# Idokorro/MiniGrid-RL

Hardware: AMD Instinct MI355X
Metric: env-steps/sec at 65k parallel envs, 1/2/4/8 MI355X; % HBM roofline (higher is better)
Workload: dtype u8

## Files before the change

### minigrid-rl_amd/csrc/mgx_device.h

```cpp
#pragma once
#ifndef MGX_HOST_SIM
#include <hip/hip_runtime.h>
#else
#include "host_sim.h"
#endif
#include <stdint.h>

#include "mgx_diag.h"

namespace mgx {

constexpr uint8_t CODE_EMPTY = 0x01;
constexpr uint8_t CODE_WALL = 2 | (5 << 4);
constexpr uint8_t CODE_GOAL = 8 | (1 << 4);
constexpr uint8_t CODE_LAVA = 9;
constexpr int T_EMPTY = 1, T_WALL = 2, T_DOOR = 4, T_KEY = 5, T_BALL = 6, T_BOX = 7,
              T_GOAL = 8, T_LAVA = 9, T_OPEN = 11;
constexpr int A_LEFT = 0, A_RIGHT = 1, A_FORWARD = 2, A_PICKUP = 3, A_DROP = 4,
              A_TOGGLE = 5, A_DONE = 6;
constexpr uint8_t NONE8 = 0xFF;

__device__ __forceinline__ int cn2idx(int cn) { return (0x403512 >> (cn * 4)) & 0xF; }

__device__ __forceinline__ uint8_t mk_code(int t, int cidx, int aux) {
// ... 276 lines not shown
#else
#define GCOUNT(G, k) do { } while (0)
#endif
#endif


template <int NW>
__device__ __forceinline__ void put(Gen<NW> &G, int x, int y, uint8_t code) {
    const int b = y * G.S + x;
    G.g[b] = code;
    if (code == CODE_EMPTY) G.occ.unset(b); else G.occ.set(b);
}

#ifndef MGX_HOST_SIM
typedef __attribute__((address_space(3))) uint64_t lds_u64;
#else
typedef uint64_t lds_u64;
#endif
constexpr int MT_PAD = MT_WG_MAX + 4;
template <int WG>
__device__ __noinline__ void mt_refill_cold(const uint64_t *__restrict__ table, uint64_t slot, lds_u64 *win) {
    const uint4 *src = reinterpret_cast<const uint4 *>(table + slot);
    static_assert(WG % 8 == 0 && WG <= MT_WG_MAX, "window loads go in fours of 16 B");
#pragma unroll
    for (int h = 0; h < WG / 8; h++) {
        const uint4 v0 = src[4 * h], v1 = src[4 * h + 1], v2 = src[4 * h + 2], v3 = src[4 * h + 3];
        lds_u64 *d = win + 8 * h;
        d[0] = (uint64_t)v0.x | ((uint64_t)v0.y << 32); d[1] = (uint64_t)v0.z | ((uint64_t)v0.w << 32);
        d[2] = (uint64_t)v1.x | ((uint64_t)v1.y << 32); d[3] = (uint64_t)v1.z | ((uint64_t)v1.w << 32);
        d[4] = (uint64_t)v2.x | ((uint64_t)v2.y << 32); d[5] = (uint64_t)v2.z | ((uint64_t)v2.w << 32);
        d[6] = (uint64_t)v3.x | ((uint64_t)v3.y << 32); d[7] = (uint64_t)v3.z | ((uint64_t)v3.w << 32);
    }
}
template <int NW>
__device__ __forceinline__ uint64_t win_group(Gen<NW> &G, uint64_t g) {
    constexpr int MT_WG = mt_wg<NW>();
    uint64_t off = g - G.gbase;
    if (off >= MT_WG) {
        GCOUNT(G, 23);
        if (g < G.tlo || g + MT_WG > G.thi) G.err |= 1u;
        mt_refill_cold<MT_WG>(G.table, g & G.rmask, (lds_u64 *)G.win);
        G.gbase = g;
        off = 0;
    }
    return G.win[off];
}
__device__ __forceinline__ uint64_t div10(uint64_t v) { return __umul64hi(v, 0xCCCCCCCCCCCCCCCDull) >> 3; }
template <int NW>
__device__ __forceinline__ void mt_sync(Gen<NW> &G) {
    const uint64_t g = div10(G.cur);
    G.go = (int)(G.cur - g * MT_FIELDS);
    G.gi = g;
    G.ga = win_group(G, g);
    G.gb = win_group(G, g + 1);
    G.gc = win_group(G, g + 2);
}
struct RbConst {
    uint64_t c1;
    uint32_t sh;
};
__device__ __forceinline__ RbConst rb_const(uint32_t n) {
    const uint32_t sh = 5u - (uint32_t)(32 - __clz(n));
    return RbConst{(uint64_t)(32u + (n << sh) - 1u) * MT_REP, sh};
}
template <int NW>
__device__ __forceinline__ int randbelow_c(Gen<NW> &G, const RbConst K);
template <int NW>
__device__ __forceinline__ int randbelow(Gen<NW> &G, uint32_t n) {
    GCOUNT(G, 24);
    if (n >= 32u) { G.err |= 8u; return 0; }
    return randbelow_c(G, rb_const(n));
}
template <int NW>
__device__ __forceinline__ int randbelow_c(Gen<NW> &G, const RbConst K) {
    const uint64_t c1 = K.c1;
    const uint32_t sh = K.sh;
    for (;;) {
        GCOUNT(G, 21);
        const int o6 = (int)__umul24((uint32_t)G.go, 6u);
        const uint64_t f = ((G.ga >> o6) | (G.gb << (60 - o6))) & MT_LOW60;
        const uint64_t acc = (c1 - f) & (32ull * MT_REP);
        const uint32_t left = G.llw - (uint32_t)(G.cur - G.astart);
        const int j = acc ? (int)(((uint32_t)__ffsll((long long)acc) - 1u - 5u) * 171u >> 10) : MT_FIELDS;
        int m = j < MT_FIELDS ? j + 1 : MT_FIELDS;
        if ((uint32_t)m > left) {
            G.cur = G.astart + G.llw;
            G.abort = true;
            return 0;
        }
        const int r = (int)(((f >> (6 * (j < MT_FIELDS ? j : 0))) & 31u) >> sh);
        G.cur += (uint64_t)m;
        G.go += m;
        if (G.go >= MT_FIELDS) {
            G.go -= MT_FIELDS;
            G.ga = G.gb;
            G.gb = G.gc;
            G.gi++;
            G.gc = win_group(G, G.gi + 2);
        }
        if (j < MT_FIELDS) return r;
    }
}
template <class GT>
__device__ __forceinline__ void mt_advance(GT &G, int m) {
    G.cur += (uint64_t)m;
    G.go += m;
    if (G.go >= MT_FIELDS) {
        G.go -= MT_FIELDS;
        G.ga = G.gb;
        G.gb = G.gc;
        G.gi++;
        G.gc = win_group(G, G.gi + 2);
    }
}
template <class GT>
__device__ __forceinline__ uint64_t randbelow_seq(GT &G, uint64_t prog, int cnt) {
    constexpr uint64_t GM = 32ull * MT_REP;
    uint64_t res = 0;
    int i = 0;
#pragma unroll 1
    while (i < cnt) {
        GCOUNT(G, 21);
        const int o6 = (int)__umul24((uint32_t)G.go, 6u);
        const uint64_t f = ((G.ga >> o6) | (G.gb << (60 - o6))) & MT_LOW60;
        uint64_t avail = GM;
        int used = MT_FIELDS;
#pragma unroll 1
        while (i < cnt) {
            const RbConst K = rb_const((uint32_t)(prog >> (5 * i)) & 31u);
            const uint64_t acc = (K.c1 - f) & avail;
            if (!acc) { used = MT_FIELDS; break; }
            const int b = __ffsll((long long)acc) - 1;
            res |= (uint64_t)((((uint32_t)(f >> (b - 5))) & 31u) >> K.sh) << (5 * i);
            avail &= ~((2ull << b) - 1ull);
            used = (int)((uint32_t)(b + 1) * 171u >> 10);
            i++;
        }
        const uint32_t left = G.llw - (uint32_t)(G.cur - G.astart);
        if ((uint32_t)used > left) {
            G.cur = G.astart + G.llw;
            G.abort = true;
            return res;
        }
        mt_advance(G, used);
    }
    return res;
}
__device__ __forceinline__ uint32_t guard10(uint64_t acc) {
    constexpr uint32_t K = (1u << 20) | (1u << 15) | (1u << 10) | (1u << 5) | 1u;
    const uint32_t lo = (uint32_t)acc >> 5, hi = (uint32_t)(acc >> 32) >> 3;
    return (((lo * K) >> 20) & 31u) | ((((hi * K) >> 20) & 31u) << 5);
}
template <int NW, typename Bad, typename Sat>
__device__ __forceinline__ void draw_cell(Gen<NW> &G, const RbConst KX, const RbConst KY, int x0, int y0, int &x, int &y,
                                          Bad bad, Sat sat ,
                                          bool has_c, const RbConst KC, int &choice) {
    constexpr uint64_t GM = 32ull * MT_REP;
    int rej = 0;
    bool need_c = has_c, have_x = false;
    uint32_t xv = 0;
#pragma unroll 1
    for (;;) {
        GCOUNT(G, 27);
        GCOUNT(G, 21);
        const int o6 = (int)__umul24((uint32_t)G.go, 6u);
        const uint64_t f = ((G.ga >> o6) | (G.gb << (60 - o6))) & MT_LOW60;
        uint32_t avail = 0x3FFu;
        if (need_c) {
            const uint32_t mc = guard10((KC.c1 - f) & GM);
            const uint32_t j = (uint32_t)__builtin_ctz(mc | 0x400u);
            choice = mc ? (int)((((uint32_t)(f >> (6u * j))) & 31u) >> KC.sh) : choice;
            avail &= ~1u << j;
            need_c = mc == 0u;
        }
        const uint32_t mx = guard10((KX.c1 - f) & GM), my = guard10((KY.c1 - f) & GM);
        bool ok;
        uint32_t jy;
#pragma unroll 1
        for (;;) {
            GCOUNT(G, 25);
            const uint32_t cx = mx & avail;
            const uint32_t jx = (uint32_t)__builtin_ctz(cx | 0x400u);
            const uint32_t xn = (((uint32_t)(f >> (6u * jx))) & 31u) >> KX.sh;
            const uint32_t av = have_x ? avail : avail & (~1u << jx);
            xv = have_x ? xv : xn;
            const uint32_t cy = my & av;
            jy = (uint32_t)__builtin_ctz(cy | 0x400u);
            x = x0 + (int)xv;
            y = y0 + (int)((((uint32_t)(f >> (6u * jy))) & 31u) >> KY.sh);
            avail = av & (~1u << jy);
            have_x = cy == 0u && (have_x || cx != 0u);
            ok = cy != 0u && !bad(x, y);
            if (ok || cy == 0u) break;
            if (++rej == SAT_PROBE && !sat()) { live_lock(G); return; }
        }
        const int used = ok ? (int)jy + 1 : MT_FIELDS;
        const uint32_t left = G.llw - (uint32_t)(G.cur - G.astart);
        if ((uint32_t)used > left) {
            G.cur = G.astart + G.llw;
            G.abort = true;
            return;
        }
        G.cur += (uint64_t)used;
        G.go += used;
        const bool rot = G.go >= MT_FIELDS;
        G.go -= rot ? MT_FIELDS : 0;
        G.ga = rot ? G.gb : G.ga;
        G.gb = rot ? G.gc : G.gb;
        G.gi += rot ? 1ull : 0ull;
        G.gc = win_group(G, G.gi + 2);
        if (ok) return;
    }
}

template <int NW>
__device__ __forceinline__ int randint(Gen<NW> &G, int a, int b) { return a + randbelow(G, (uint32_t)(b - a + 1)); }
template <int NW>
__device__ __forceinline__ bool choice_bool(Gen<NW> &G) { return randbelow(G, 2) == 0; }

template <int NW>
__device__ __forceinline__ bool next2door(const Gen<NW> &G, int x, int y) {
    if constexpr (NW == 4) {
        return is_door(G.g[y * G.S + x - 1]) || is_door(G.g[y * G.S + x + 1]) ||
               is_door(G.g[(y - 1) * G.S + x]) || is_door(G.g[(y + 1) * G.S + x]);
    } else {
        return G.dn.test(y * G.S + x);
    }
}
template <int NW>
__device__ __forceinline__ bool occupied(const Gen<NW> &G, int b) {
    if constexpr (NW == 4) return G.g[b] != CODE_EMPTY;
    else return G.occ.test(b);
}

constexpr uint32_t OBJ_KEYFLAG = 1u << 24;
template <int NW>
__device__ __forceinline__ void add_obj(Gen<NW> &G, int t, int cname, int x, int y, uint32_t flags = 0) {
    const bool full = G.nobjs >= MAX_OBJS;
    G.err |= full ? 8u : 0u;
    G.tmask |= full ? 0u : 1u << t;
    const bool first_goal = !full && t == T_GOAL && G.goalx < 0;
    G.goalx = first_goal ? x : G.goalx;
    G.goaly = first_goal ? y : G.goaly;
    if (!full)
        G.objs[G.nobjs++] = (uint32_t)t | ((uint32_t)(cname & 15) << 4) | ((uint32_t)x << 8) | ((uint32_t)y << 16) | flags;
}

template <int NW>
__device__ __forceinline__ void draw_free_cell(Gen<NW> &G, int &px, int &py) {
    for (uint32_t it = 0;; ++it) {
        GCOUNT(G, 22);
        if (it > PCG_LOOP_LIMIT) { G.err |= 4u; px = 1; py = 1; return; }
        int x, y;
        pcg_cell(G.pcg, G.S, x, y);
        if (occupied(G, y * G.S + x)) continue;
        if (x == G.ax && y == G.ay) continue;
        px = x; py = y;
        return;
    }
}
template <int NW>
__device__ __forceinline__ void place_agent(Gen<NW> &G) {
    G.ax = -1; G.ay = -1;
    int x, y;
    draw_free_cell(G, x, y);
    G.ax = x; G.ay = y;
    G.adir = pcg_integers(G.pcg, 0, 4);
}

__device__ __forceinline__ int nth_set_bit(uint32_t m, int r) {
    int pos = 0, c;
    c = __popc(m & 0xFFFFu); if (r >= c) { r -= c; m >>= 16; pos += 16; }
    c = __popc(m & 0xFFu);   if (r >= c) { r -= c; m >>= 8;  pos += 8; }
    c = __popc(m & 0xFu);    if (r >= c) { r -= c; m >>= 4;  pos += 4; }
    c = __popc(m & 0x3u);    if (r >= c) { r -= c; m >>= 2;  pos += 2; }
    c = (int)(m & 1u);       if (r >= c) { pos += 1; }
    return pos;
}
template <int NW>
__device__ __forceinline__ int mask_choice(Gen<NW> &G, uint32_t m) {
    return nth_set_bit(m, randbelow(G, (uint32_t)__popc(m)));
}

template <int NW>
__device__ __forceinline__ void live_lock(Gen<NW> &G) {
    G.cur = G.astart + G.llw;
    G.abort = true;
}

template <int NW>
__device__ __forceinline__ void place_key(Gen<NW> &G, int x0, int x1, int y0, int y1, int gx, int gy, bool chk_agent,
                                          int ox, int oy, int cname, bool kib, int *kx, int *ky) {
    int x, y, rej = 0;
    for (;;) {
        x = randint(G, x0, x1);
        y = randint(G, y0, y1);
        if (G.abort) return;
        const bool bad = (x == gx && y == gy) || (chk_agent && x == G.ax && y == G.ay) || (x == ox && y == oy) ||
                         next2door(G, x, y);
        if (!bad) break;
        if (++rej == SAT_PROBE) {
            bool sat = false;
            for (int xx = x0; xx <= x1 && !sat; xx++)
                for (int yy = y0; yy <= y1 && !sat; yy++)
                    sat = !((xx == gx && yy == gy) || (chk_agent && xx == G.ax && yy == G.ay) ||
                            (xx == ox && yy == oy) || next2door(G, xx, yy));
            if (!sat) { live_lock(G); return; }
        }
    }
    const int cidx = cn2idx(cname);
    if (kib) { put(G, x, y, mk_code(T_BOX, cidx, 1)); add_obj(G, T_BOX, cname, x, y, OBJ_KEYFLAG); }
    else { put(G, x, y, mk_code(T_KEY, cidx, 0)); add_obj(G, T_KEY, cname, x, y, OBJ_KEYFLAG); }
    if (kx) { *kx = x; *ky = y; }
}

template <int NW>
__device__ __forceinline__ void place_objects(Gen<NW> &G, uint32_t &oc, const int *types, int n, int x0, int x1,
                                              int y0, int y1) {
    for (int k = 0; k < n; k++) {
        if (oc == 0) { G.err |= 8u; return; }
        const int b = mask_choice(G, oc);
        if (G.abort) return;
        oc &= ~(1u << b);
        const int t = types[b / 6], cname = b % 6;
        int x, y, rej = 0;
        for (;;) {
            x = randint(G, x0, x1);
            y = randint(G, y0, y1);
            if (G.abort) return;
            const bool bad = occupied(G, y * G.S + x) || (x == G.ax && y == G.ay) || next2door(G, x, y);
            if (!bad) break;
            if (++rej == SAT_PROBE) {
                bool sat = false;
                for (int xx = x0; xx <= x1 && !sat; xx++)
                    for (int yy = y0; yy <= y1 && !sat; yy++)
                        sat = !(occupied(G, yy * G.S + xx) || (xx == G.ax && yy == G.ay) || next2door(G, xx, yy));
                if (!sat) { live_lock(G); return; }
            }
        }
        put(G, x, y, mk_code(t, cn2idx(cname), 0));
        add_obj(G, t, cname, x, y);
    }
}

__device__ __forceinline__ int door_code(int cname, bool locked, bool open) {
    return open ? mk_code(T_OPEN, cn2idx(cname), 0) : mk_code(T_DOOR, cn2idx(cname), locked ? 1 : 0);
}

template <int NW>
__device__ __forceinline__ void put_door(Gen<NW> &G, int x, int y, uint8_t code) {
    put(G, x, y, code);
    const int S = G.S, b = y * S + x;
    if (x > 0) G.dn.set(b - 1);
    if (x < S - 1) G.dn.set(b + 1);
    if (y > 0) G.dn.set(b - S);
    if (y < S - 1) G.dn.set(b + S);
}

template <int NW>
__device__ __forceinline__ uint32_t bits_row(const Bits<NW> &B, int y, int S) {
    const int b = y * S;
    uint64_t v = b < 64 ? (B.w0 >> b) : 0ull;
    if (NW > 1) {
        if (b >= 64) v = B.w1 >> (b - 64);
        else if (b + S > 64) v |= B.w1 << (64 - b);
    }
    return (uint32_t)v & ((1u << S) - 1u);
}
template <int NW>
__device__ __forceinline__ bool rect_has_free(const Gen<NW> &G, int x0, int x1, int y0, int y1, bool use_occ,
                                              int ax, int ay, int bx, int by, int cx, int cy) {
    if constexpr (NW == 4) {
        return true;
    } else {
        const uint32_t rowmask = ((1u << (x1 - x0 + 1)) - 1u) << x0;
        bool sat = false;
        for (int y = y0; y <= y1; y++) {
            uint32_t bad = bits_row(G.dn, y, G.S);
            if (use_occ) bad |= bits_row(G.occ, y, G.S);
            if (ay == y && ax >= 0) bad |= 1u << ax;
            if (by == y && bx >= 0) bad |= 1u << bx;
            if (cy == y && cx >= 0) bad |= 1u << cx;
            sat |= (rowmask & ~bad) != 0;
        }
        return sat;
    }
}


__device__ __forceinline__ void door_geom(int nr, int d, int mid, int S, bool &horiz, int &lo, int &hi) {
    if (nr == 2) { horiz = false; lo = 1; hi = S - 2; return; }
    if (nr == 3) {
        horiz = d == 0;
        lo = d == 2 ? mid + 1 : 1;
        hi = d == 2 ? S - 2 : mid - 1;
        return;
    }
    horiz = d < 2;
    const bool upper_half = (d == 0 || d == 2);
    lo = upper_half ? 1 : mid + 1;
    hi = upper_half ? mid - 1 : S - 2;
}

__device__ __forceinline__ int room_of(int nr, int x, int y, int mid) {
    const bool left = x < mid, up = y < mid;
    if (nr == 2) return left ? 0 : 1;
    if (nr == 3) return left ? (up ? 0 : 1) : 2;
    return left ? (up ? 0 : 1) : (up ? 2 : 3);
}

__device__ __forceinline__ void room_rect(int nr, int r, int mid, int S, int &x0, int &x1, int &y0, int &y1) {
    const bool left = (nr == 2) ? r == 0 : r <= 1;
    const bool full_h = nr == 2 || (nr == 3 && r == 2);
    const bool up = (r == 0) || (nr == 4 && r == 2);
    x0 = left ? 1 : mid + 1; x1 = left ? mid - 1 : S - 2;
    y0 = full_h ? 1 : (up ? 1 : mid + 1); y1 = full_h ? S - 2 : (up ? mid - 1 : S - 2);
}

__device__ __forceinline__ void key_spec(int nr, int r, int ar, int &kA, int &kB, bool &chk) {
    kA = -1; kB = -1; chk = (r == ar);
    if (nr == 2) { if (r == ar) kA = 0; return; }
    if (nr == 3) {
        if (r != ar) return;
        if (r == 0) { kA = 1; kB = 0; }
        else if (r == 1) { kA = 2; kB = 0; }
        else { kA = 2; kB = 1; }
        return;
    }
    const int HL = 0, HR = 1, VU = 2, VL = 3;
    if (r == 0) {
        if (ar == 0) { kA = VU; kB = HL; } else if (ar == 1) kA = VU; else if (ar == 2) kA = HL;
    } else if (r == 1) {
        if (ar == 1) { kA = VL; kB = HL; } else if (ar == 3) kA = HL; else if (ar == 0) kA = VL;
    } else if (r == 2) {
        if (ar == 2) { kA = VU; kB = HR; } else if (ar == 3) kA = VU; else if (ar == 0) kA = HR;
    } else {
        if (ar == 3) { kA = VL; kB = HR; } else if (ar == 1) kA = HR; else if (ar == 2) kA = VL;
    }
}

__device__ const int MULTI_TYPES[3] = {T_KEY, T_BALL, T_BOX};

struct Prefix {
    int nr, rc;
    uint32_t dinfo;
    uint32_t dpos;
    uint32_t dopen;
};
template <class GT>
__device__ __forceinline__ void prefix_draws(GT &G, int S, bool draw_cmd, bool ado, Prefix &P) {
    const uint64_t r = randbelow_seq(G, draw_cmd ? (4ull | (3ull << 5)) : 3ull, draw_cmd ? 2 : 1);
    P.rc = draw_cmd ? (int)(r & 31) : 0;
    P.nr = 2 + (int)((draw_cmd ? r >> 5 : r) & 31);
    P.dinfo = P.dpos = P.dopen = 0;
    if (G.abort || (MGX_GEN_SKIP & 8)) return;
    const int nr = P.nr, mid = S / 2, ndoors = nr == 2 ? 1 : nr;
    uint64_t prog = 0;
    int cnt = 0;
#pragma unroll 1
    for (int d = 0; d < ndoors; d++) {
        prog |= (uint64_t)(6 - d) << (5 * cnt++);
        if (!ado) prog |= 2ull << (5 * cnt++);
        prog |= 2ull << (5 * cnt++);
    }
    const uint64_t dr = randbelow_seq(G, prog, cnt);
    if (G.abort) return;
    uint32_t dc = 0x3Fu;
#pragma unroll 1
    for (int d = 0, k = 0; d < ndoors; d++) {
        const int col = nth_set_bit(dc, (int)(dr >> (5 * k++)) & 31);
        dc &= ~(1u << col);
        const bool lk = ado ? false : ((dr >> (5 * k++)) & 31) == 0;
        const bool kib = ((dr >> (5 * k++)) & 31) == 0;
        P.dinfo |= (uint32_t)(col | (lk << 3) | (kib << 4)) << (8 * d);
    }
    prog = 0;
    cnt = 0;
#pragma unroll 1
    for (int d = 0; d < ndoors; d++) {
        bool horiz; int lo, hi;
        door_geom(nr, d, mid, S, horiz, lo, hi);
        prog |= (uint64_t)(hi - lo + 1) << (5 * cnt++);
        if (ado) prog |= 2ull << (5 * cnt++);
    }
    const uint64_t pr = randbelow_seq(G, prog, (MGX_GEN_SKIP & 2) ? 0 : cnt);
    if (G.abort) return;
#pragma unroll 1
    for (int d = 0, k = 0; d < ((MGX_GEN_SKIP & 2) ? 0 : ndoors); d++) {
        P.dpos |= (uint32_t)((pr >> (5 * k++)) & 15) << (4 * d);
        if (ado) P.dopen |= (uint32_t)(((pr >> (5 * k++)) & 31) == 0) << d;
    }
}
constexpr int PFX_LOOK = 320;
__host__ __device__ __forceinline__ uint64_t pfx_pack(const Prefix &P, uint32_t adv, uint32_t tag) {
    uint64_t r = (uint64_t)(adv & 0xFF) | ((uint64_t)(tag & 0xFF) << 8) | ((uint64_t)(P.nr - 2) << 16) |
                 ((uint64_t)(P.rc & 3) << 18);
    for (int d = 0; d < 4; d++)
        r |= (uint64_t)(((P.dinfo >> (8 * d)) & 31) | (((P.dpos >> (4 * d)) & 15) << 5) | (((P.dopen >> d) & 1) << 9))
             << (20 + 10 * d);
    return r;
}
__host__ __device__ __forceinline__ void pfx_unpack(uint64_t r, Prefix &P) {
    P.nr = 2 + (int)((r >> 16) & 3);
    P.rc = (int)((r >> 18) & 3);
    P.dinfo = P.dpos = P.dopen = 0;
    for (int d = 0; d < 4; d++) {
        const uint32_t f = (uint32_t)(r >> (20 + 10 * d)) & 0x3FFu;
        P.dinfo |= (f & 31u) << (8 * d);
        P.dpos |= ((f >> 5) & 15u) << (4 * d);
        P.dopen |= ((f >> 9) & 1u) << d;
    }
}
constexpr int MT_SB_WORDS = 3120;
constexpr int MT_SB_GROUPS = MT_SB_WORDS / MT_FIELDS;
constexpr int MT_SLIDE_MAX_SB = 64;
__host__ __device__ __forceinline__ int mt_slide_superblocks(unsigned long long hi, unsigned long long need_lo,
                                                             unsigned long long want_hi,
                                                             unsigned long long ring_groups) {
    int nsb = 0;
    while (nsb < MT_SLIDE_MAX_SB && hi + (unsigned long long)nsb * MT_SB_GROUPS < want_hi &&
           hi + (unsigned long long)(nsb + 1) * MT_SB_GROUPS <= need_lo + ring_groups)
        nsb++;
    return nsb;
}
struct PfxWindow {
    unsigned long long zero_lo, rec_lo, rec_hi;
    unsigned long long next_done;
    unsigned long long strides;
};
__host__ __device__ __forceinline__ PfxWindow pfx_window(unsigned long long rec_done, unsigned long long hi,
                                                         unsigned long long ring_words, unsigned long long threads,
                                                         unsigned long long look) {
    const unsigned long long top = hi * (unsigned long long)MT_FIELDS;
    const unsigned long long held = top > ring_words ? top - ring_words : 0ull;
    PfxWindow w;
    w.rec_hi = top > look ? top - look : 0ull;
    w.rec_lo = rec_done > held ? rec_done : held;
    if (w.rec_hi < w.rec_lo) w.rec_hi = w.rec_lo;
    w.zero_lo = w.rec_lo;
    if (rec_done < held) {
        const unsigned long long kept = w.rec_hi > ring_words ? w.rec_hi - ring_words : 0ull;
        w.zero_lo = rec_done > kept ? rec_done : kept;
    }
    w.next_done = w.rec_hi;
    w.strides = (w.rec_hi - w.rec_lo + threads - 1) / threads;
    return w;
}

template <int NW>
__device__ __forceinline__ void gen_rooms(Gen<NW> &G, const Prefix &P) {
    const int S = G.S, mid = S / 2, nr = P.nr;
    if (MGX_GEN_SKIP & 8) { G.ax = 1; G.ay = 1; put(G, S - 2, S - 2, CODE_GOAL); add_obj(G, T_GOAL, 15, S - 2, S - 2); return; }
    for (int i = 1; i < S - 1; i++) put(G, mid, i, CODE_WALL);
    if (nr == 3) for (int i = 1; i < mid; i++) put(G, i, mid, CODE_WALL);
    if (nr == 4) for (int i = 1; i < S - 1; i++) put(G, i, mid, CODE_WALL);
    const int ndoors = nr == 2 ? 1 : nr;
    const bool ado = G.all_doors_open;
    const uint32_t dinfo = P.dinfo;
    uint32_t oc = 0x3FFFFu;
#pragma unroll 1
    for (int d = 0; d < ndoors; d++) {
        const uint32_t di = dinfo >> (8 * d);
        const int col = di & 7;
        if ((di >> 3) & 1) { oc &= ~(1u << col); if ((di >> 4) & 1) oc &= ~(1u << (12 + col)); }
    }
    GSTAMP(G, 11);
#pragma unroll 1
    for (int d = 0; d < ((MGX_GEN_SKIP & 2) ? 0 : ndoors); d++) {
        bool horiz; int lo, hi;
        door_geom(nr, d, mid, S, horiz, lo, hi);
        const int v = lo + (int)((P.dpos >> (4 * d)) & 15);
        const int x = horiz ? v : mid, y = horiz ? mid : v;
        const uint32_t di = dinfo >> (8 * d);
        const bool open = ado && ((P.dopen >> d) & 1);
        put_door(G, x, y, (uint8_t)door_code(di & 7, (di >> 3) & 1, open));
        add_obj(G, T_DOOR, di & 7, x, y);
    }
    GSTAMP(G, 12);
    if (G.abort) return;
    int gx = 1, gy = 1;
    if (MGX_GEN_SKIP & 4) {
        gx = 1; gy = 1; put(G, gx, gy, CODE_GOAL); add_obj(G, T_GOAL, 15, gx, gy); G.ax = S - 2; G.ay = S - 2;
    } else {
        bool agent = false;
        int gcell = -1;
        if constexpr (NW <= 2) {
#pragma unroll 1
            for (uint32_t it = 0;; ++it) {
                GCOUNT(G, 22);
                if (it > 2 * PCG_LOOP_LIMIT) { G.err |= 4u; G.ax = 1; G.ay = 1; break; }
                int x, y;
                pcg_cell(G.pcg, S, x, y);
                const int b = y * S + x;
                Bits<NW> rejm = G.occ;
                rejm.w0 |= agent ? 0ull : G.dn.w0;
                if (NW > 1) rejm.w1 |= agent ? 0ull : G.dn.w1;
                if (rejm.test(b)) continue;
                if (agent) { G.ax = x; G.ay = y; break; }
                gx = x; gy = y; gcell = b;
                G.occ.set(b);
                agent = true;
            }
        } else {
#pragma unroll 1
            for (uint32_t it = 0;; ++it) {
                GCOUNT(G, 22);
                if (it > 2 * PCG_LOOP_LIMIT) { G.err |= 4u; G.ax = 1; G.ay = 1; break; }
                int x, y;
                pcg_cell(G.pcg, S, x, y);
                const int b = y * S + x;
                if (occupied(G, b) || b == gcell) continue;
                if (agent) { G.ax = x; G.ay = y; break; }
                if (next2door(G, x, y)) continue;
                gx = x; gy = y; gcell = b;
                agent = true;
            }
        }
        if (gcell >= 0) {
            put(G, gx, gy, CODE_GOAL);
            add_obj(G, T_GOAL, 15, gx, gy);
        }
        G.adir = pcg_integers(G.pcg, 0, 4);
    }
    GSTAMP(G, 13);
    const int gr = room_of(nr, gx, gy, mid), ar = room_of(nr, G.ax, G.ay, mid);
    const int n_left = G.num_objects / 2, n_right = G.num_objects - n_left;
    int c0, c1, c2, c3;
    if (nr == 2) { c0 = n_left; c1 = n_right; c2 = c3 = 0; }
    else if (nr == 3) { c0 = n_left / 2; c1 = n_left - c0; c2 = n_right; c3 = 0; }
    else { c0 = n_left / 2; c1 = n_left - c0; c2 = n_right / 2; c3 = n_right - c2; }
    uint32_t keymask = 0;
    uint32_t npack = 0;
    uint32_t kspec = 0;
#pragma unroll
    for (int r = 0; r < 4; r++) {
        int kA, kB;
        bool chk;
        key_spec(nr, r, ar, kA, kB, chk);
        kspec |= (uint32_t)(kA & 3) << (4 * r) | (uint32_t)(kB & 3) << (4 * r + 2) | (uint32_t)chk << (16 + r);
        const bool a = r < nr && kA >= 0 && ((dinfo >> (8 * kA + 3)) & 1);
        const bool b = r < nr && kB >= 0 && ((dinfo >> (8 * kB + 3)) & 1);
        keymask |= (uint32_t)a << (2 * r) | (uint32_t)b << (2 * r + 1);
        const int ndec = (int)a + (int)b + (int)(gr == r);
        int n;
        if (r == 0) { c0 -= ndec; n = c0; }
        else if (r == 1) { c1 -= ndec; n = (nr == 2) ? c1 : c0; }
        else if (r == 2) { c2 -= ndec; n = c2; }
        else { c3 -= ndec; n = c3; }
        npack |= (uint32_t)(n > 0 ? n : 0) << (8 * r);
    }
    uint64_t reps = 0;
    if (NW == 1)
        for (int i = 0; i < S; i++) reps |= 1ull << (i * S);
    uint64_t todo = 0;
#pragma unroll
    for (int rr = 0; rr < 4; rr++)
        todo |= (uint64_t)(((keymask >> (2 * rr)) & 3u) | ((((1u << ((npack >> (8 * rr)) & 0xFF)) - 1u) & 0x3FFFu) << 2))
                << (16 * rr);
    if (MGX_GEN_SKIP & 1) return;
    int kx = -1, ky = -1;
#pragma unroll 1
    while (todo) {
        GCOUNT(G, 20);
        GSTAMP(G, 19);
        GSTAMP(G, 16);
        const int slot = (int)__builtin_ctzll(todo);
        const int r = slot >> 4, phase = min(slot & 15, 2);
        int x0, x1, y0, y1;
        room_rect(nr, r, mid, S, x0, x1, y0, y1);
        const bool is_key = phase < 2;
        int cname, ot = T_KEY, ox = -1, oy = -1;
        bool chk = false, kib = false;
        if (is_key) {
            chk = (kspec >> (16 + r)) & 1;
            const uint32_t di = dinfo >> (8 * ((kspec >> (4 * r + 2 * phase)) & 3));
            cname = di & 7;
            kib = (di >> 4) & 1;
            if (phase == 1 && ((keymask >> (2 * r)) & 1)) { ox = kx; oy = ky; }
        } else {
            if (oc == 0) { G.err |= 8u; break; }
        }
        const bool has_c = !is_key && !(MGX_GEN_SKIP & 32);
        const RbConst kc_ = rb_const(is_key ? 1u : (uint32_t)__popc(oc));
        int choice = 0;
        const int ex0 = is_key ? gx : G.ax, ey0 = is_key ? gy : G.ay;
        const int ex1 = (is_key && !chk) ? -1 : G.ax, ey1 = (is_key && !chk) ? -1 : G.ay;
        const RbConst kx_ = rb_const((uint32_t)(x1 - x0 + 1)), ky_ = rb_const((uint32_t)(y1 - y0 + 1));
        int x, y;
        GSTAMP(G, 17);
        if constexpr (NW <= 2) {
            Bits<NW> bad = G.dn;
            if (!is_key) { bad.w0 |= G.occ.w0; if (NW > 1) bad.w1 |= G.occ.w1; }
            bad.set(ey0 * S + ex0);
            if (ex1 >= 0) bad.set(ey1 * S + ex1);
            if (ox >= 0) bad.set(oy * S + ox);
            bool sat;
            if constexpr (NW == 1) {
                const uint64_t rows = reps & (((1ull << ((y1 + 1) * S)) - 1ull) & ~((1ull << (y0 * S)) - 1ull));
                sat = ((rows * (uint64_t)(((1u << (x1 - x0 + 1)) - 1u) << x0)) & ~bad.w0) != 0;
            } else {
                sat = rect_has_free(G, x0, x1, y0, y1, !is_key, ex0, ey0, ex1, ey1, ox, oy);
            }
            if (!sat) {
                live_lock(G);
                return;
            }
            draw_cell(G, kx_, ky_, x0, y0, x, y, [&](int cx, int cy) { return bad.test(cy * S + cx); },
                      [] { return true; }, has_c, kc_, choice);
            if (G.abort) return;
        } else {
            const auto bad = [&](int cx, int cy) {
                return (cx == ex0 && cy == ey0) || (cx == ex1 && cy == ey1) || (cx == ox && cy == oy) ||
                       (!is_key && occupied(G, cy * S + cx)) || next2door(G, cx, cy);
            };
            draw_cell(G, kx_, ky_, x0, y0, x, y, bad, [&] {
                for (int xx = x0; xx <= x1; xx++)
                    for (int yy = y0; yy <= y1; yy++)
                        if (!bad(xx, yy)) return true;
                return false;
            }, has_c, kc_, choice);
            if (G.abort) return;
        }
        if (!is_key) {
            const int b = (MGX_GEN_SKIP & 32) ? __ffs(oc) - 1 : nth_set_bit(oc, choice);
            oc &= ~(1u << b);
            ot = MULTI_TYPES[b / 6];
            cname = b % 6;
        }
        GSTAMP(G, 18);
        const int cidx = cn2idx(cname);
        const int t = is_key ? (kib ? T_BOX : T_KEY) : ot;
        put(G, x, y, mk_code(t, cidx, (is_key && kib) ? 1 : 0));
        add_obj(G, t, cname, x, y, is_key ? OBJ_KEYFLAG : 0u);
        if (phase == 0) { kx = x; ky = y; }
        todo &= todo - 1;
    }
    GSTAMP(G, 14);
}

template <int NW>
__device__ __forceinline__ int gen_multi(Gen<NW> &G) {
    const bool draw_cmd = G.cfg_mission < 0;
    Prefix P;
    if (G.phave) {
        pfx_unpack(G.prec, P);
    } else {
#if MGX_GEN_PREFIX2
        { const uint64_t c0_ = G.cur; prefix_draws(G, G.S, draw_cmd, G.all_doors_open != 0, P); G.cur = c0_; G.abort = false; mt_sync(G); }
#endif
        prefix_draws(G, G.S, draw_cmd, G.all_doors_open != 0, P);
        if (G.abort) return 0;
    }
    const int cmd = draw_cmd ? (P.rc == 3 ? 5 : P.rc) : G.cfg_mission;
    GSTAMP(G, 10);
    gen_rooms(G, P);
    return cmd;
}

__device__ const int GTO_T[4] = {T_KEY, T_BALL, T_BOX, T_DOOR};
__device__ const int GTG_T[4] = {T_BOX, T_DOOR, T_KEY, T_BALL};
__device__ const int OPN_T[2] = {T_BOX, T_DOOR};
__device__ const int PKP_T[3] = {T_KEY, T_BOX, T_BALL};

template <int NW, bool EXT>
__device__ __forceinline__ int gen_single(Gen<NW> &G) {
    const int *types;
    int ntypes, cmd;
    bool goal = false;
    const bool full = EXT && G.problem == 1;
    if constexpr (EXT) {
        switch (G.problem) {
            case 1: types = GTO_T; ntypes = 4; cmd = -1; goal = true; break;
            case 2: types = GTO_T; ntypes = 4; cmd = 0; break;
            case 3: types = GTG_T; ntypes = 4; cmd = 5; goal = true; break;
            case 4: types = OPN_T; ntypes = 2; cmd = 1; break;
            case 6: types = GTO_T; ntypes = 4; cmd = 3; goal = true; break;
            case 7: types = GTO_T; ntypes = 4; cmd = 4; break;
            default: types = PKP_T; ntypes = 3; cmd = 2; break;
        }
    } else {
        switch (G.problem) {
            case 2: types = GTO_T; ntypes = 4; cmd = 0; break;
            case 3: types = GTG_T; ntypes = 4; cmd = 5; goal = true; break;
            case 4: types = OPN_T; ntypes = 2; cmd = 1; break;
            default: types = PKP_T; ntypes = 3; cmd = 2; break;
        }
    }
    uint32_t oc = (1u << (ntypes * 6)) - 1u;
    const int nplace = full ? 24 : G.num_objects;
    for (int k = 0; k < nplace; k++) {
        if (oc == 0) { G.err |= 8u; break; }
        const int b = full ? k : mask_choice(G, oc);
        if (G.abort) return 0;
        oc &= ~(1u << b);
        const int t = types[b / 6], cname = b % 6;
        int x, y;
        draw_free_cell(G, x, y);
        put(G, x, y, mk_code(t, cn2idx(cname), 0));
        add_obj(G, t, cname, x, y);
    }
    if (goal) {
        int x, y;
        draw_free_cell(G, x, y);
        put(G, x, y, CODE_GOAL);
        add_obj(G, T_GOAL, 15, x, y);
    }
    place_agent(G);
    if (full) cmd = pcg_integers(G.pcg, 0, 6);
    return cmd;
}

struct ResetOut {
    uint8_t tx, ty, ta, mission_id;
    int livelocks;
    uint64_t range;
};

template <int NW>
__device__ __forceinline__ bool in_objs(const Gen<NW> &G, int x, int y) {
    const uint32_t key = (uint32_t)x << 8 | (uint32_t)y << 16;
    bool hit = false;
    for (int k = 0; k < G.nobjs; k++) hit |= (G.objs[k] & 0xFFFF00u) == key;
    return hit;
}

template <int NW>
__device__ __forceinline__ void place_obstacles(Gen<NW> &G) {
    const int S = G.S, mid = S / 2;
#pragma unroll 1
    for (int k = 0; k < G.n_obstacles; k++) {
        if (G.problem == 0) {
            int x, y, rej = 0;
            for (;;) {
                x = randint(G, 1, S - 2);
                y = randint(G, 1, S - 2);
                if (G.abort) return;
                const bool bad = x == mid || y == mid || in_objs(G, x, y) || (x == G.ax && y == G.ay) ||
                                 next2door(G, x, y);
                if (!bad) break;
                if (++rej == SAT_PROBE) {
                    bool sat = false;
                    for (int xx = 1; xx <= S - 2 && !sat; xx++)
                        for (int yy = 1; yy <= S - 2 && !sat; yy++)
                            sat = !(xx == mid || yy == mid || in_objs(G, xx, yy) || (xx == G.ax && yy == G.ay) ||
                                    next2door(G, xx, yy));
                    if (!sat) { live_lock(G); return; }
                }
            }
            put(G, x, y, CODE_LAVA);
        } else {
            const bool lava = randbelow(G, 2) == 0;
            if (G.abort) return;
            int x, y;
            draw_free_cell(G, x, y);
            put(G, x, y, lava ? CODE_LAVA : CODE_WALL);
        }
    }
}

template <int NW>
__device__ __forceinline__ uint64_t move_range(const Gen<NW> &G, int d) {
    const int S = G.S;
    uint64_t rg = (uint64_t)d;
    for (int k = 1; k < S - 1; k++) {
        int v;
        bool ok;
        if (d == 0) { v = 1; while (v < S - 1 && G.g[k * S + v] != CODE_EMPTY) v++; ok = v < S - 1; }
        else if (d == 1) { v = S - 2; while (v > 0 && G.g[k * S + v] != CODE_EMPTY) v--; ok = v > 0; }
        else if (d == 2) { v = 1; while (v < S - 1 && G.g[v * S + k] != CODE_EMPTY) v++; ok = v < S - 1; }
        else { v = S - 2; while (v > 0 && G.g[v * S + k] != CODE_EMPTY) v--; ok = v > 0; }
        if (ok) rg |= (uint64_t)v << (4 * k);
    }
    return rg;
}
__device__ __forceinline__ bool in_move_range(uint64_t rg, int ax, int ay) {
    const bool rows = (rg & 3) < 2;
    const int idx = rows ? ay : ax, coord = rows ? ax : ay;
    const int ent = (int)((rg >> (4 * idx)) & 15);
    return ent != 0 && ent == coord;
}

__device__ __forceinline__ void apply_vis(uint8_t *fr) {
    uint32_t T[7];
#pragma unroll
    for (int vy = 0; vy < 7; vy++) {
        uint32_t t = 0;
#pragma unroll
        for (int vx = 0; vx < 7; vx++) {
// ... 136 lines not shown
```

Baseline: 2.563 billion.

## Flatten object placement into single loop to reduce warp divergence

Splits the rejection-sampling draw into a single-pass helper and restructures the object-placement loop into one flat state machine. Each iteration either sets up a new placement task or performs one draw pass, so lanes at different stages can stay converged inside a single loop. It also precomputes room geometry masks, replacing per-object rectangle computation and the constant-memory type table with branchless arithmetic. The cost is more live state held in registers and some extra select logic per iteration.

```diff
diff --git a/minigrid-rl_amd/csrc/mgx_device.h b/minigrid-rl_amd/csrc/mgx_device.h
--- a/minigrid-rl_amd/csrc/mgx_device.h
+++ b/minigrid-rl_amd/csrc/mgx_device.h
@@ -452,65 +452,67 @@
     return (((lo * K) >> 20) & 31u) | ((((hi * K) >> 20) & 31u) << 5);
 }
 template <int NW, typename Bad, typename Sat>
+__device__ __forceinline__ bool cell_pass(Gen<NW> &G, const RbConst KX, const RbConst KY, int x0, int y0, int &x, int &y,
+                                          Bad bad, Sat sat ,
+                                          const RbConst KC, int &choice, bool &need_c, bool &have_x, uint32_t &xv,
+                                          int &rej) {
+    constexpr uint64_t GM = 32ull * MT_REP;
+    GCOUNT(G, 27);
+    GCOUNT(G, 21);
+    const int o6 = (int)__umul24((uint32_t)G.go, 6u);
+    const uint64_t f = ((G.ga >> o6) | (G.gb << (60 - o6))) & MT_LOW60;
+    uint32_t avail = 0x3FFu;
+    if (need_c) {
+        const uint32_t mc = guard10((KC.c1 - f) & GM);
+        const uint32_t j = (uint32_t)__builtin_ctz(mc | 0x400u);
+        choice = mc ? (int)((((uint32_t)(f >> (6u * j))) & 31u) >> KC.sh) : choice;
+        avail &= ~1u << j;
+        need_c = mc == 0u;
+    }
+    const uint32_t mx = guard10((KX.c1 - f) & GM), my = guard10((KY.c1 - f) & GM);
+    bool ok, dead = false;
+    uint32_t jy;
+#pragma unroll 1
+    for (;;) {
+        GCOUNT(G, 25);
+        const uint32_t cx = mx & avail;
+        const uint32_t jx = (uint32_t)__builtin_ctz(cx | 0x400u);
+        const uint32_t xn = (((uint32_t)(f >> (6u * jx))) & 31u) >> KX.sh;
+        const uint32_t av = have_x ? avail : avail & (~1u << jx);
+        xv = have_x ? xv : xn;
+        const uint32_t cy = my & av;
+        jy = (uint32_t)__builtin_ctz(cy | 0x400u);
+        x = x0 + (int)xv;
+        y = y0 + (int)((((uint32_t)(f >> (6u * jy))) & 31u) >> KY.sh);
+        avail = av & (~1u << jy);
+        have_x = cy == 0u && (have_x || cx != 0u);
+        ok = cy != 0u && !bad(x, y);
+        if (ok || cy == 0u) break;
+        if (++rej == SAT_PROBE && !sat()) { dead = true; break; }
+    }
+    const int used = ok ? (int)jy + 1 : MT_FIELDS;
+    const uint32_t left = G.llw - (uint32_t)(G.cur - G.astart);
+    const bool stop = dead || (uint32_t)used > left;
+    const int adv = stop ? 0 : used;
+    G.cur = stop ? G.astart + G.llw : G.cur + (uint64_t)used;
+    G.abort |= stop;
+    G.go += adv;
+    const bool rot = G.go >= MT_FIELDS;
+    G.go -= rot ? MT_FIELDS : 0;
+    G.ga = rot ? G.gb : G.ga;
+    G.gb = rot ? G.gc : G.gb;
+    G.gi += rot ? 1ull : 0ull;
+    G.gc = win_group(G, G.gi + 2);
+    return ok && !stop;
+}
+template <int NW, typename Bad, typename Sat>
 __device__ __forceinline__ void draw_cell(Gen<NW> &G, const RbConst KX, const RbConst KY, int x0, int y0, int &x, int &y,
-                                          Bad bad, Sat sat ,
-                                          bool has_c, const RbConst KC, int &choice) {
-    constexpr uint64_t GM = 32ull * MT_REP;
+                                          Bad bad, Sat sat, bool has_c, const RbConst KC, int &choice) {
     int rej = 0;
     bool need_c = has_c, have_x = false;
     uint32_t xv = 0;
 #pragma unroll 1
-    for (;;) {
-        GCOUNT(G, 27);
-        GCOUNT(G, 21);
-        const int o6 = (int)__umul24((uint32_t)G.go, 6u);
-        const uint64_t f = ((G.ga >> o6) | (G.gb << (60 - o6))) & MT_LOW60;
-        uint32_t avail = 0x3FFu;
-        if (need_c) {
-            const uint32_t mc = guard10((KC.c1 - f) & GM);
-            const uint32_t j = (uint32_t)__builtin_ctz(mc | 0x400u);
-            choice = mc ? (int)((((uint32_t)(f >> (6u * j))) & 31u) >> KC.sh) : choice;
-            avail &= ~1u << j;
-            need_c = mc == 0u;
-        }
-        const uint32_t mx = guard10((KX.c1 - f) & GM), my = guard10((KY.c1 - f) & GM);
-        bool ok;
-        uint32_t jy;
-#pragma unroll 1
-        for (;;) {
-            GCOUNT(G, 25);
-            const uint32_t cx = mx & avail;
-            const uint32_t jx = (uint32_t)__builtin_ctz(cx | 0x400u);
-            const uint32_t xn = (((uint32_t)(f >> (6u * jx))) & 31u) >> KX.sh;
-            const uint32_t av = have_x ? avail : avail & (~1u << jx);
-            xv = have_x ? xv : xn;
-            const uint32_t cy = my & av;
-            jy = (uint32_t)__builtin_ctz(cy | 0x400u);
-            x = x0 + (int)xv;
-            y = y0 + (int)((((uint32_t)(f >> (6u * jy))) & 31u) >> KY.sh);
-            avail = av & (~1u << jy);
-            have_x = cy == 0u && (have_x || cx != 0u);
-            ok = cy != 0u && !bad(x, y);
-            if (ok || cy == 0u) break;
-            if (++rej == SAT_PROBE && !sat()) { live_lock(G); return; }
-        }
-        const int used = ok ? (int)jy + 1 : MT_FIELDS;
-        const uint32_t left = G.llw - (uint32_t)(G.cur - G.astart);
-        if ((uint32_t)used > left) {
-            G.cur = G.astart + G.llw;
-            G.abort = true;
-            return;
-        }
-        G.cur += (uint64_t)used;
-        G.go += used;
-        const bool rot = G.go >= MT_FIELDS;
-        G.go -= rot ? MT_FIELDS : 0;
-        G.ga = rot ? G.gb : G.ga;
-        G.gb = rot ? G.gc : G.gb;
-        G.gi += rot ? 1ull : 0ull;
-        G.gc = win_group(G, G.gi + 2);
-        if (ok) return;
-    }
+    while (!cell_pass(G, KX, KY, x0, y0, x, y, bad, sat, KC, choice, need_c, have_x, xv, rej) && !G.abort) {}
 }
 
 template <int NW>
@@ -668,21 +670,13 @@
     return (uint32_t)v & ((1u << S) - 1u);
 }
 template <int NW>
-__device__ __forceinline__ bool rect_has_free(const Gen<NW> &G, int x0, int x1, int y0, int y1, bool use_occ,
-                                              int ax, int ay, int bx, int by, int cx, int cy) {
+__device__ __forceinline__ bool rect_has_free(const Bits<NW> &bad, int x0, int wx, int y0, int wy, int S) {
     if constexpr (NW == 4) {
         return true;
     } else {
-        const uint32_t rowmask = ((1u << (x1 - x0 + 1)) - 1u) << x0;
+        const uint32_t rowmask = ((1u << wx) - 1u) << x0;
         bool sat = false;
-        for (int y = y0; y <= y1; y++) {
-            uint32_t bad = bits_row(G.dn, y, G.S);
-            if (use_occ) bad |= bits_row(G.occ, y, G.S);
-            if (ay == y && ax >= 0) bad |= 1u << ax;
-            if (by == y && bx >= 0) bad |= 1u << bx;
-            if (cy == y && cx >= 0) bad |= 1u << cx;
-            sat |= (rowmask & ~bad) != 0;
-        }
+        for (int y = y0; y < y0 + wy; y++) sat |= (rowmask & ~bits_row(bad, y, S)) != 0;
         return sat;
     }
 }
@@ -709,12 +703,8 @@
     return left ? (up ? 0 : 1) : (up ? 2 : 3);
 }
 
-__device__ __forceinline__ void room_rect(int nr, int r, int mid, int S, int &x0, int &x1, int &y0, int &y1) {
-    const bool left = (nr == 2) ? r == 0 : r <= 1;
-    const bool full_h = nr == 2 || (nr == 3 && r == 2);
-    const bool up = (r == 0) || (nr == 4 && r == 2);
-    x0 = left ? 1 : mid + 1; x1 = left ? mid - 1 : S - 2;
-    y0 = full_h ? 1 : (up ? 1 : mid + 1); y1 = full_h ? S - 2 : (up ? mid - 1 : S - 2);
+__device__ __forceinline__ uint32_t room_classes(int nr) {
+    return nr == 2 ? 0x54u : (nr == 3 ? 0x520u : 0x3120u);
 }
 
 __device__ __forceinline__ void key_spec(int nr, int r, int ar, int &kA, int &kB, bool &chk) {
@@ -738,8 +728,6 @@
         if (ar == 3) { kA = VL; kB = HR; } else if (ar == 1) kA = HR; else if (ar == 2) kA = VL;
     }
 }
-
-__device__ const int MULTI_TYPES[3] = {T_KEY, T_BALL, T_BOX};
 
 struct Prefix {
     int nr, rc;
@@ -949,9 +937,20 @@
         else { c3 -= ndec; n = c3; }
         npack |= (uint32_t)(n > 0 ? n : 0) << (8 * r);
     }
-    uint64_t reps = 0;
-    if (NW == 1)
+    const int wa = mid - 1, wb = S - 2 - mid;
+    const RbConst KA = rb_const((uint32_t)wa), KB = rb_const((uint32_t)wb), KF = rb_const((uint32_t)(S - 2));
+    uint64_t colA = 0, colB = 0, rowA = 0, rowB = 0, rowF = 0;
+    if (NW == 1) {
+        uint64_t reps = 0;
         for (int i = 0; i < S; i++) reps |= 1ull << (i * S);
+        colA = reps * (uint64_t)(((1u << wa) - 1u) << 1);
+        colB = reps * (uint64_t)(((1u << wb) - 1u) << (mid + 1));
+        rowA = ((1ull << (mid * S)) - 1ull) & ~((1ull << S) - 1ull);
+        rowB = ((1ull << ((S - 1) * S)) - 1ull) & ~((1ull << ((mid + 1) * S)) - 1ull);
+        rowF = ((1ull << ((S - 1) * S)) - 1ull) & ~((1ull << S) - 1ull);
+    }
+    const uint32_t geo = room_classes(nr);
+    const int bgoal = gy * S + gx, bagent = G.ay * S + G.ax;
     uint64_t todo = 0;
 #pragma unroll
     for (int rr = 0; rr < 4; rr++)
@@ -959,81 +958,98 @@
                 << (16 * rr);
     if (MGX_GEN_SKIP & 1) return;
     int kx = -1, ky = -1;
+    bool fresh = true, objtask = false;
+    int x0 = 0, y0 = 0, wx = 0, wy = 0, e0 = -1, e1 = -1, e2 = -1;
+    RbConst KX = KA, KY = KA, KC = KA;
+    Bits<NW> bad;
+    bad.clear();
+    bool need_c = false, have_x = false;
+    uint32_t xv = 0;
+    int rej = 0, choice = 0;
 #pragma unroll 1
     while (todo) {
-        GCOUNT(G, 20);
         GSTAMP(G, 19);
-        GSTAMP(G, 16);
-        const int slot = (int)__builtin_ctzll(todo);
-        const int r = slot >> 4, phase = min(slot & 15, 2);
-        int x0, x1, y0, y1;
-        room_rect(nr, r, mid, S, x0, x1, y0, y1);
-        const bool is_key = phase < 2;
-        int cname, ot = T_KEY, ox = -1, oy = -1;
-        bool chk = false, kib = false;
-        if (is_key) {
-            chk = (kspec >> (16 + r)) & 1;
-            const uint32_t di = dinfo >> (8 * ((kspec >> (4 * r + 2 * phase)) & 3));
-            cname = di & 7;
-            kib = (di >> 4) & 1;
-            if (phase == 1 && ((keymask >> (2 * r)) & 1)) { ox = kx; oy = ky; }
-        } else {
-            if (oc == 0) { G.err |= 8u; break; }
-        }
-        const bool has_c = !is_key && !(MGX_GEN_SKIP & 32);
-        const RbConst kc_ = rb_const(is_key ? 1u : (uint32_t)__popc(oc));
-        int choice = 0;
-        const int ex0 = is_key ? gx : G.ax, ey0 = is_key ? gy : G.ay;
-        const int ex1 = (is_key && !chk) ? -1 : G.ax, ey1 = (is_key && !chk) ? -1 : G.ay;
-        const RbConst kx_ = rb_const((uint32_t)(x1 - x0 + 1)), ky_ = rb_const((uint32_t)(y1 - y0 + 1));
-        int x, y;
+        if (fresh) {
+            GCOUNT(G, 20);
+            const int slot = (int)__builtin_ctzll(todo);
+            const int r = slot >> 4, ph = slot & 15;
+            const bool is_key = ph < 2;
+            const uint32_t gq = geo >> (4 * r);
+            const bool xb = gq & 1u, yb = gq & 2u, yf = gq & 4u;
+            x0 = xb ? mid + 1 : 1;
+            wx = xb ? wb : wa;
+            KX.c1 = xb ? KB.c1 : KA.c1; KX.sh = xb ? KB.sh : KA.sh;
+            y0 = yb ? mid + 1 : 1;
+            wy = yf ? S - 2 : (yb ? wb : wa);
+            KY.c1 = yf ? KF.c1 : (yb ? KB.c1 : KA.c1); KY.sh = yf ? KF.sh : (yb ? KB.sh : KA.sh);
+            const bool none = !is_key && oc == 0u;
+            G.err |= none ? 8u : 0u;
+            KC = rb_const(is_key ? 1u : (uint32_t)__popc(oc));
+            const bool chk = (kspec >> (16 + r)) & 1u;
+            const bool other = ph == 1 && ((keymask >> (2 * r)) & 1u);
+            objtask = !is_key;
+            e0 = is_key ? bgoal : -1;
+            e1 = (!is_key || chk) ? bagent : -1;
+            e2 = other ? ky * S + kx : -1;
+            bool sat = true;
+            if constexpr (NW <= 2) {
+                bad = G.dn;
+                bad.w0 |= is_key ? 0ull : G.occ.w0;
+                if (NW > 1) bad.w1 |= is_key ? 0ull : G.occ.w1;
+                bad.set(e0);
+                bad.set(e1);
+                bad.set(e2);
+                if constexpr (NW == 1) sat = ((xb ? colB : colA) & (yf ? rowF : (yb ? rowB : rowA)) & ~bad.w0) != 0;
+                else sat = rect_has_free(bad, x0, wx, y0, wy, S);
+            }
+            if (!none && !sat) live_lock(G);
+            todo = (none || !sat) ? 0ull : todo;
+            need_c = !is_key && !(MGX_GEN_SKIP & 32);
+            have_x = false;
+            xv = 0;
+            rej = 0;
+            choice = 0;
+            fresh = false;
+        }
         GSTAMP(G, 17);
-        if constexpr (NW <= 2) {
-            Bits<NW> bad = G.dn;
-            if (!is_key) { bad.w0 |= G.occ.w0; if (NW > 1) bad.w1 |= G.occ.w1; }
-            bad.set(ey0 * S + ex0);
-            if (ex1 >= 0) bad.set(ey1 * S + ex1);
-            if (ox >= 0) bad.set(oy * S + ox);
-            bool sat;
-            if constexpr (NW == 1) {
-                const uint64_t rows = reps & (((1ull << ((y1 + 1) * S)) - 1ull) & ~((1ull << (y0 * S)) - 1ull));
-                sat = ((rows * (uint64_t)(((1u << (x1 - x0 + 1)) - 1u) << x0)) & ~bad.w0) != 0;
+        if (todo) {
+            int x, y;
+            bool ok;
+            if constexpr (NW <= 2) {
+                ok = cell_pass(G, KX, KY, x0, y0, x, y, [&](int cx, int cy) { return bad.test(cy * S + cx); },
+                               [] { return true; }, KC, choice, need_c, have_x, xv, rej);
             } else {
-                sat = rect_has_free(G, x0, x1, y0, y1, !is_key, ex0, ey0, ex1, ey1, ox, oy);
+                const auto badc = [&](int cx, int cy) {
+                    const int b = cy * S + cx;
+                    return b == e0 || b == e1 || b == e2 || (objtask && occupied(G, b)) || next2door(G, cx, cy);
+                };
+                ok = cell_pass(G, KX, KY, x0, y0, x, y, badc, [&] {
+                    for (int xx = x0; xx < x0 + wx; xx++)
+                        for (int yy = y0; yy < y0 + wy; yy++)
+                            if (!badc(xx, yy)) return true;
+                    return false;
+                }, KC, choice, need_c, have_x, xv, rej);
             }
-            if (!sat) {
-                live_lock(G);
-                return;
+            GSTAMP(G, 18);
+            if (ok) {
+                const int slot = (int)__builtin_ctzll(todo);
+                const int r = slot >> 4, ph = slot & 15;
+                const bool is_key = ph < 2;
+                const uint32_t di = dinfo >> (8 * ((kspec >> (4 * r + 2 * (ph & 1))) & 3));
+                const int b = (MGX_GEN_SKIP & 32) ? __ffs(oc) - 1 : nth_set_bit(oc, choice);
+                oc &= is_key ? ~0u : ~(1u << b);
+                const int cname = is_key ? (int)(di & 7u) : b % 6;
+                const bool kib = is_key && ((di >> 4) & 1u);
+                const int t = is_key ? (kib ? T_BOX : T_KEY) : (b < 6 ? T_KEY : (b < 12 ? T_BALL : T_BOX));
+                put(G, x, y, mk_code(t, cn2idx(cname), kib ? 1 : 0));
+                add_obj(G, t, cname, x, y, is_key ? OBJ_KEYFLAG : 0u);
+                kx = ph == 0 ? x : kx;
+                ky = ph == 0 ? y : ky;
+                todo &= todo - 1;
+                fresh = true;
             }
-            draw_cell(G, kx_, ky_, x0, y0, x, y, [&](int cx, int cy) { return bad.test(cy * S + cx); },
-                      [] { return true; }, has_c, kc_, choice);
-            if (G.abort) return;
-        } else {
-            const auto bad = [&](int cx, int cy) {
-                return (cx == ex0 && cy == ey0) || (cx == ex1 && cy == ey1) || (cx == ox && cy == oy) ||
-                       (!is_key && occupied(G, cy * S + cx)) || next2door(G, cx, cy);
-            };
-            draw_cell(G, kx_, ky_, x0, y0, x, y, bad, [&] {
-                for (int xx = x0; xx <= x1; xx++)
-                    for (int yy = y0; yy <= y1; yy++)
-                        if (!bad(xx, yy)) return true;
-                return false;
-            }, has_c, kc_, choice);
-            if (G.abort) return;
-        }
-        if (!is_key) {
-            const int b = (MGX_GEN_SKIP & 32) ? __ffs(oc) - 1 : nth_set_bit(oc, choice);
-            oc &= ~(1u << b);
-            ot = MULTI_TYPES[b / 6];
-            cname = b % 6;
-        }
-        GSTAMP(G, 18);
-        const int cidx = cn2idx(cname);
-        const int t = is_key ? (kib ? T_BOX : T_KEY) : ot;
-        put(G, x, y, mk_code(t, cidx, (is_key && kib) ? 1 : 0));
-        add_obj(G, t, cname, x, y, is_key ? OBJ_KEYFLAG : 0u);
-        if (phase == 0) { kx = x; ky = y; }
-        todo &= todo - 1;
+            todo = G.abort ? 0ull : todo;
+        }
     }
     GSTAMP(G, 14);
 }
```

New measurement: 2.637 billion (median of 6 runs). +2.9%, better.
